# hkbharath/MARL-MASS

Measured on AMD Instinct MI355X. Metric: agent-steps/sec (whole node), MASS CBF shield on, 65536 envs x 8 CAVs, higher is better.
Workload: dtype f64

## Files before the change

### marl-mass_amd/csrc/mm_kernels.hip

```cpp
#include <hip/hip_runtime.h>
#include <math.h>
#include <stdio.h>
#include <string.h>

#include <type_traits>

#include "mm_device.h"
#include "mm_div.h"
#include "mm_handle.h"
#define MM_COUNTS_FN __host__ __device__ inline
#include "../../include/mm_counts.h"
#include "../../include/mm_policy_wide.h"

using namespace mm;

struct DevCfg {
  int env_kind, shield, nsub, T, action_masking, auto_reset, obs_f64, N, E, debug_flags, n_hdv;
  double dt, collision_reward, high_speed_reward, headway_cost, headway_time, merging_lane_cost;
  double rs_lo, rs_hi, eta, tau;
  double inv_dt, rs_span, rs_ispan, rs_span2, rs_ispan2;
  int agent_reward;
  int steer_vel;
  int *err;
  int traffic_density, mixed_traffic, num_cav;
// ... 11 lines not shown
  uint64_t *seeds;
  long long A;
  int E, N;
};

enum {
  SW_CPSI, SW_ACCN,
  SW_AX, SW_AY, SW_AH, SW_ACPSI, SW_AGVX, SW_ASTEER, SW_ASPSI,
  SW_BX, SW_BY, SW_BH, SW_BCPSI, SW_BGVX, SW_BSTEER, SW_BSPSI,
  SW_ACC,
  SW_F_COUNT
};
enum { SW_WPK, SW_APK, SW_BPK, SW_META, SW_RES, SW_CLS, SW_I_COUNT };
struct SweepBuf {
  double *F;
  int *I;
  uint8_t *order;
  uint8_t *envf;
  uint8_t *urgent;
  long long Ep;
  int N;
};
MM_DEV double &sw_f(const SweepBuf &sb, int f, int a, long long e) { return sb.F[((long long)f * sb.N + a) * sb.Ep + e]; }
MM_DEV int &sw_i(const SweepBuf &sb, int f, int a, long long e) { return sb.I[((long long)f * sb.N + a) * sb.Ep + e]; }

enum { PB_SIN, PB_COS, PB_KX, PB_KY, PB_KH, PB_F_COUNT };
constexpr int kPoseWritten = 0x200;
struct PoseBuf {
  double *F;
  int *code;
};

#ifndef MM_TU
#define MM_TU 0
#endif

#ifdef MM_STAMPS
#define MM_STAMP_WAVES (1 << 16)
__device__ unsigned long long g_stamps_w[MM_STAMP_WAVES * 16];
__device__ unsigned long long g_stamps_s[4096 * 8];
#define SSTAMP(k)                                                                        \
  do {                                                                                   \
    unsigned long long _t = __builtin_amdgcn_s_memtime();                                \
    if ((threadIdx.x & 63) == (k)) _t_acc += _t - _t_last;                               \
    _t_last = __builtin_amdgcn_s_memtime();                                              \
  } while (0)
#define SCOUNT(k) do { if ((threadIdx.x & 63) == (k)) _t_acc += 1; } while (0)
#define STAMP(k)                                                                         \
  do {                                                                                   \
    unsigned long long _t = __builtin_amdgcn_s_memtime();                                \
    if ((threadIdx.x & 63) == (k)) _t_acc += _t - _t_last;                               \
    _t_last = __builtin_amdgcn_s_memtime();                                              \
  } while (0)
#else
#define STAMP(k) do {} while (0)
#define SSTAMP(k) do {} while (0)
#define SCOUNT(k) do {} while (0)
#endif

template <int KIND> constexpr bool kIdm = KIND == MM_ENV_HDV_V1;

struct Veh {
  double x, y, h, v, tspeed;
  double act_steer, act_acc, safe_steer, safe_acc, gvx;
  double h1x, h1vx, h2x, h2vx;
  double sang;
  int lane, tlane, sidx, crashed, hl, flags, hist_len;
  int kind;
  bool present;
};

MM_DEV int lane_id() { return threadIdx.x & 63; }
MM_DEV double shfl_d(double v, int src) { return __shfl(v, src, 64); }
MM_DEV int shfl_i(int v, int src) { return __shfl(v, src, 64); }

template <int M>
MM_DEV int dppx_i(int v) {
  static_assert(M >= 1 && M <= 15, "xor mask within a 16-lane DPP row");
  if constexpr (M == 1) return __builtin_amdgcn_update_dpp(0, v, 0xB1, 0xF, 0xF, false);
  else if constexpr (M == 2) return __builtin_amdgcn_update_dpp(0, v, 0x4E, 0xF, 0xF, false);
  else if constexpr (M == 3) return __builtin_amdgcn_update_dpp(0, v, 0x1B, 0xF, 0xF, false);
  else if constexpr (M == 7) return __builtin_amdgcn_update_dpp(0, v, 0x141, 0xF, 0xF, false);
  else if constexpr (M == 8) return __builtin_amdgcn_update_dpp(0, v, 0x128, 0xF, 0xF, false);
  else if constexpr (M == 15) return __builtin_amdgcn_update_dpp(0, v, 0x140, 0xF, 0xF, false);
  else if constexpr (M < 7) return dppx_i<7>(dppx_i<7 - M>(v));
  else if constexpr (M < 12) return dppx_i<8>(dppx_i<M - 8>(v));
  else return dppx_i<15>(dppx_i<15 - M>(v));
}
template <int M>
MM_DEV double dppx_d(double v) {
  long long b = __double_as_longlong(v);
  int lo = dppx_i<M>((int)(unsigned)(b & 0xFFFFFFFFll)), hi = dppx_i<M>((int)(b >> 32));
  return __longlong_as_double(((long long)hi << 32) | (unsigned)lo);
}
template <int M, int G, class F>
MM_DEV void for_partners_impl(F &f) {
  if constexpr (M < G) {
    f(std::integral_constant<int, M>{});
    for_partners_impl<M + 1, G>(f);
  }
}
template <int G, class F>
MM_DEV void for_partners(F f) { for_partners_impl<1, G>(f); }

template <int G> constexpr bool kPow2 = (G & (G - 1)) == 0;
#ifndef MM_ROUNDS_LITE
#define MM_ROUNDS_LITE 1
#endif
constexpr bool kRoundsLite = MM_ROUNDS_LITE != 0;
#ifndef MM_VETO_PRIOR
// ... 1032 lines not shown
#ifndef MM_MIN_WAVES
#define MM_MIN_WAVES 2
#endif
#ifndef MM_NONE_WAVES
#define MM_NONE_WAVES 3
#endif
#ifndef MM_NONE_WIDE_G
#define MM_NONE_WIDE_G 99
#endif
#ifndef MM_IPM_WAVES
#define MM_IPM_WAVES 2
#endif
#ifndef MM_IPM_CAV_WAVES
#define MM_IPM_CAV_WAVES 2
#endif
#ifndef MM_IPM_WIDE_WAVES
#define MM_IPM_WIDE_WAVES 1
#endif
#ifndef MM_SPLIT_WAVES
#define MM_SPLIT_WAVES 2
#endif
template <int G, int SHIELD, bool MIXED>
#ifndef MM_GENERAL_NONE_WAVES
#define MM_GENERAL_NONE_WAVES 3
#endif
constexpr int step_min_waves(bool ipm = false) { return SHIELD == MM_SHIELD_NONE ? (G >= MM_NONE_WIDE_G ? 2 : (MIXED ? MM_GENERAL_NONE_WAVES : MM_NONE_WAVES)) : (ipm ? (G >= 6 ? MM_IPM_WIDE_WAVES : (MIXED ? MM_IPM_WAVES : MM_IPM_CAV_WAVES)) : MM_MIN_WAVES); }
template <int G, int KIND, int SHIELD, bool MIXED, bool IPM = false, bool TRACE = false, bool SPLIT = false>
#ifndef MM_STEP_BLOCK
#define MM_STEP_BLOCK 64
#endif
__global__ __launch_bounds__(MM_STEP_BLOCK, (SPLIT ? MM_SPLIT_WAVES : step_min_waves<G, SHIELD, MIXED>(IPM))) void step_kernel(DevCfg c, DevState st, const int32_t *__restrict__ actions,
                                                   MMStepOut out, double *metrics, SweepBuf sb, int kb, PoseBuf pb) {
  constexpr bool IDM = kIdm<KIND>;
  constexpr bool LC = (KIND == MM_ENV_V1) || IDM;
  constexpr bool SHIELDED = LC && (SHIELD != MM_SHIELD_NONE);
  static_assert(!IDM || (MIXED && SHIELD == MM_SHIELD_NONE && !IPM && !SPLIT), "hdv-v1: general unshielded kernels only");
  constexpr bool MASS = (SHIELD == MM_SHIELD_MASS);
  static_assert(!IPM || SHIELDED, "the IPM mode lives in shielded kernels");
  static_assert(!SPLIT || IPM, "the split form exists for the interior-point kernels");
#ifdef MM_SERIAL_ALL
  constexpr bool kSerialOnly = true || IPM;
#else
#ifdef MM_SERIAL_MASS
  constexpr bool kSerialOnly = MIXED || MASS || IPM;
#else
  constexpr bool kSerialOnly = MIXED;
#endif
#endif
  constexpr bool kSine = SHIELDED && !SPLIT && !MIXED && !IPM && !kSerialOnly && kPow2<G> && G <= 8;
#ifndef MM_CARRY_POSE
#define MM_CARRY_POSE 1
#endif
  constexpr bool kCarry = kSine && MM_CARRY_POSE != 0;
  static_assert(kPow2<G> || MM_STEP_BLOCK == 64, "rotation layouts: one wave per workgroup");
  const long long gtid = (long long)blockIdx.x * blockDim.x + threadIdx.x;
  constexpr int kTail = kPow2<G> ? 64 : (64 / G) * G;
  const bool tail = lane_id() >= kTail;
  const int gb = kPow2<G> ? (lane_id() & ~(G - 1)) : (tail ? kTail - G : lane_id() - lane_id() % G);
  const int a = kPow2<G> ? (int)(gtid % G) : lane_id() - gb;
  const long long e = kPow2<G> ? gtid / G : (tail ? (long long)st.E : (gtid >> 6) * (64 / G) + lane_id() / G);
  const bool valid = e < st.E && a < st.N;
  const long long i = e * st.N + a;
  const long long A = st.A;
  const double dt = c.dt;

#ifdef MM_STAMPS
  unsigned long long _t_last = __builtin_amdgcn_s_memtime(), _t_acc = 0;
#endif
  Veh v;
  const bool sv = MIXED && KIND == MM_ENV_V1 && c.steer_vel != 0;
  int steps = 0, time = 0, n_merge = 0, episode = 0;
  int car_code = 0;
  long long car_kx = 0, car_ky = 0, car_kh = 0;
  double car_s = 0.0, car_c = 1.0;
  if constexpr (kCarry) {
    if (valid) {
      car_kx = __double_as_longlong(pb.F[PB_KX * A + i]); car_ky = __double_as_longlong(pb.F[PB_KY * A + i]);
      car_kh = __double_as_longlong(pb.F[PB_KH * A + i]);
      car_s = pb.F[PB_SIN * A + i]; car_c = pb.F[PB_COS * A + i]; car_code = pb.code[i];
    }
  }
  load_veh(st, i, valid, v, sv);
  if (e < st.E) {
    steps = st.I[MM_E_STEPS * st.E + e]; time = st.I[MM_E_TIME * st.E + e];
  }
  if (!MIXED && v.kind == 2) v.kind = 1;
  if (IDM && v.present) v.kind = 2;
  const bool hdv = MIXED && v.kind == 2;
  const bool ctrl = IDM ? v.present : (v.present && !hdv);
  const bool ctrl_x = IDM ? false : ctrl;
  int action = (!IDM && valid && ctrl) ? actions[i] : 1;
  if ((unsigned)action > 4u) {
    if (!SPLIT || kb == 0) atomicOr(c.err, MM_LATCH_BAD_ACTION);
    action = 1;
  }
  const unsigned present_bits = group_ballot<G>(v.present, gb);
  const unsigned ctrl_bits = group_ballot<G>(ctrl, gb);
  const int n_veh = __popc(present_bits), n_ctrl = __popc(ctrl_bits);
  if (!SPLIT || kb == 0) steps += 1;

  double cpsi = 1.0, spsi = 0.0;
  double st_t = __builtin_nan("");
  int pk_self = v.lane;
  bool carried = false;
  if constexpr (kCarry) {
    const bool hit = car_kx == __double_as_longlong(v.x) && car_ky == __double_as_longlong(v.y) && car_kh == __double_as_longlong(v.h) &&
                     (car_code >> 8) == ((kPoseWritten >> 8) | (MASS ? 1 : 0)) && (car_code & 7) == v.lane;
    carried = !__any(v.present && !hit);
    if (carried && v.present) { spsi = car_s; cpsi = car_c; pk_self = car_code & 0xFF; }
  }
  if (!carried) {
    if (v.present) mmm_sincos(v.h, &spsi, &cpsi);
    if (SHIELDED && v.present) pk_self = pose_code(v.lane, next_lane(v.lane, v.x, v.y), MASS ? corner_flags(v.x, v.y, spsi, cpsi, v.lane) : 0);
  }

  enum { C_B = 0, C_H1X = 8, C_H1VX, C_H2X, C_H2VX, C_SSTEER, C_SACC, C_TSPEED, C_A = 15, C_GU0 = 23, C_GU1 = 24, C_PRE = 25, C_MSGW = 29 };
  constexpr bool kMailbox = G <= 8 || !kPow2<G>;
  constexpr bool kPackMsg = !kPow2<G>;
  constexpr int kColdB = kMailbox ? (kPackMsg ? 29 : 30) : 25;
  constexpr bool kRoomy = false;
  constexpr int C_CPSI = kColdB + G - 1, C_GVX = C_CPSI + 1;
  constexpr int kColdN = !SHIELDED ? 15 : (kSerialOnly ? 23 : kColdB + G - 1 + (kRoomy ? 2 : 0));
  static_assert(kColdN * MM_STEP_BLOCK * 8 >= (MM_STEP_BLOCK / 64) * 64 * 30 * 4, "the obs staging must fit in the cold slots");
  __shared__ double s_cold[kColdN][MM_STEP_BLOCK];
  const int tid = threadIdx.x;
  auto cold_i = [&](int slot, int col) -> int & { return ((int *)&s_cold[slot][col])[0]; };
  if (LC) {
    s_cold[C_H1X][tid] = v.h1x; s_cold[C_H1VX][tid] = v.h1vx; s_cold[C_H2X][tid] = v.h2x; s_cold[C_H2VX][tid] = v.h2vx;
    s_cold[C_SSTEER][tid] = v.safe_steer; s_cold[C_SACC][tid] = v.safe_acc;
  }
  s_cold[C_TSPEED][tid] = v.tspeed;
  if constexpr (kRoomy) { s_cold[C_CPSI][tid] = cpsi; s_cold[C_GVX][tid] = v.gvx; }
  auto CPSI = [&]() -> double { if constexpr (kRoomy) return s_cold[C_CPSI][tid]; else return cpsi; };
  auto GVX = [&]() -> double { if constexpr (kRoomy) return s_cold[C_GVX][tid]; else return v.gvx; };
  bool env_active = IDM ? n_veh > 0 : n_ctrl > 0;
  if constexpr (SPLIT) {
    if (kb > 0) env_active = e < st.E && sb.envf[e] != 0;
  }
  STAMP(0);
  const int k_lo = SPLIT ? (kb > 0 ? kb - 1 : 0) : 0, k_hi = SPLIT ? (kb < c.nsub ? kb : c.nsub - 1) : c.nsub - 1;
  for (int k = k_lo; k <= k_hi; k++) {
    const bool head = !SPLIT || k == kb, tail = !SPLIT || k != kb;
    const bool live = env_active && v.present;
    QpTrace qt = {0, __builtin_nan(""), __builtin_nan(""), __builtin_nan(""), __builtin_nan(""),
                  __builtin_nan(""), __builtin_nan(""), __builtin_nan("")};
    int rank = 0;
    if ((SHIELDED || MIXED) && head) {
      for_partners<G>([&](auto mc) {
        constexpr int m = decltype(mc)::value;
        double px = px_d<m, G>(v.x, a);
        bool pp = px_i<m, G>((int)live, a) != 0;
        rank += (pp && (px > v.x || (px == v.x && pidx<m, G>(a) < a))) ? 1 : 0;
      });
    }
    if (head) v.tspeed = s_cold[C_TSPEED][tid];
    if (live && !hdv && head) {
      if (time % c.nsub == 0) hl_act<KIND>(v, action);
    }
    const int tl_pre = v.tlane;
    if (live && !hdv && head) controlled_act<!MIXED, kSine>(v, -1, sv, st_t);
    if (head) s_cold[C_TSPEED][tid] = v.tspeed;
    if constexpr (MIXED) { STAMP(1); }
    if constexpr (MIXED) {
      if (head && __any(hdv && live)) {
        const bool acting = hdv && live && !v.crashed;
        double koff = 0.0, koff_obst = 0.0;
        if (__any(acting && v.lane == MM_LANE_KB0)) {
          koff = kSineAmp * mmm_sin(kSinePuls * (v.x - lane_sx(MM_LANE_KB0)) + kSinePhase);
          koff_obst = kSineAmp * mmm_sin(kSinePuls * (kObstX - lane_sx(MM_LANE_KB0)) + kSinePhase);
        }
        Body self = {true, false, v.x, v.y, v.h, v.v, v.tspeed, v.lane, spsi, cpsi, koff};
        const double s_me = v.x - lane_sx(v.lane);
        NbSel n0 = {0, 0, -1, -1}, n1 = {0, 0, -1, -1};
        const LaneFrame lf0 = lane_frame(v.lane);
        if (acting && lane_after_end(v.tlane, v.x)) v.tlane = next_lane(v.tlane, v.x, v.y);
        const int my_tl = v.tlane;
        const bool lc_branch = v.lane != my_tl;
        const bool same_road = lane_road(v.lane) == lane_road(my_tl);
        const bool timer_due = !lc_branch && (1.0 < v.gvx);
        const int side = v.lane == MM_LANE_BC0 ? MM_LANE_BC1 : (v.lane == MM_LANE_BC1 ? MM_LANE_BC0 : -1);
        const bool try_mobil = acting && timer_due && side >= 0 && lane_reachable(side < 0 ? 0 : side, v.x, v.y);
        const int sl = side < 0 ? 0 : side;
        const double s_side = v.x - lane_sx(sl);
        const LaneFrame lf1 = lane_frame(sl);
        unsigned abort_mask = 0;
        for_partners<G>([&](auto mc) {
          constexpr int m = decltype(mc)::value;
          const int p = pidx<m, G>(a);
          const bool bp = px_i<m, G>((int)live, a) != 0;
          const double bx = px_d<m, G>(v.x, a), by = px_d<m, G>(v.y, a), bk = px_d<m, G>(koff, a);
          if (acting) {
            neighbour_update(lf0, s_me, bp, bx, by, bk, p, n0);
            if (try_mobil) neighbour_update(lf1, s_side, bp, bx, by, bk, p, n1);
          }
          if (__any(acting && lc_branch && same_road)) {
            Body b = {bp, false, bx, by, 0.0, px_d<m, G>(v.v, a), 0.0, px_i<m, G>(v.lane, a), px_d<m, G>(spsi, a), px_d<m, G>(cpsi, a), bk};
            if (acting && lc_branch && same_road && b.present && b.lane != my_tl) {
              const double sx = lane_sx(v.lane);
              const double d = (b.x - sx) - (v.x - sx);
              if (0 < d && d < desired_gap(self, b)) abort_mask |= 1u << p;
            }
          }
        });
        if constexpr (MIXED) { STAMP(3); }
        if (acting) {
          neighbour_update(lf0, s_me, true, kObstX, kObstY, koff_obst, 99, n0);
          if (try_mobil) neighbour_update(lf1, s_side, true, kObstX, kObstY, koff_obst, 99, n1);
        }
        auto fetch = [&](int idx, bool full) {
          Body r = {};
          const int src = gb + ((idx >= 0 && idx < G) ? idx : 0);
          r.x = shfl_d(v.x, src); r.v = shfl_d(v.v, src); r.sh = shfl_d(spsi, src); r.ch = shfl_d(cpsi, src);
          if (full) { r.tspeed = shfl_d(v.tspeed, src); r.lane = shfl_i(v.lane, src); }
          r.present = idx >= 0;
          if (idx == 99) { r.is_object = true; r.x = kObstX; r.v = 0.0; r.sh = 0.0; r.ch = 1.0; r.tspeed = 0.0; r.lane = 0; }
          return r;
        };
        const Body front0 = fetch(acting ? n0.i_front : -1, false);
        Body front1 = {}, rear1 = {};
        if (__any(try_mobil)) { front1 = fetch(try_mobil ? n1.i_front : -1, false); rear1 = fetch(try_mobil ? n1.i_rear : -1, true); }
        const double acc_f0 = acting ? idm_acceleration(self, front0) : 0.0;
        bool mobil_go = false;
        if (try_mobil) {
          const double nf_pred = idm_acceleration(rear1, self);
          if (!(nf_pred < -9.0)) {
            const double jerk = idm_acceleration(self, front1) - acc_f0 + 0.0;
            mobil_go = !(jerk < 0.1);
          }
        }
        if constexpr (MIXED) { STAMP(4); }
        if (acting && timer_due) v.gvx = 0;
        int tl_post = acting ? (lc_branch ? my_tl : (mobil_go ? side : my_tl)) : v.tlane;
        for (int round = 0; round <= st.N; round++) {
          bool hit = false;
          for_partners<G>([&](auto mc) {
            constexpr int m = decltype(mc)::value;
            const int p = pidx<m, G>(a);
            const int pk = px_i<m, G>(rank | tl_pre << 4 | tl_post << 8, a);
            const int p_tl = ((pk & 15) < rank) ? ((pk >> 8) & 7) : ((pk >> 4) & 7);
            hit = hit || (((abort_mask >> p) & 1u) && p_tl == my_tl);
          });
          const int nxt = (acting && lc_branch) ? ((same_road && hit) ? v.lane : my_tl) : tl_post;
          const bool changed = nxt != tl_post;
          tl_post = nxt;
          if (!__any(changed)) break;
        }
        if constexpr (MIXED) { STAMP(5); }
        if (acting) {
          v.tlane = tl_post;
          v.act_acc = clipd(acc_f0, -6.0, 6.0);
        }
      }
      if (head && live && (!hdv || !v.crashed)) steer_lane(v, sv && !hdv, st_t);
      if (head && hdv && live) v.gvx += dt;
    }
    if (live && head) clip_actions(v, LC && !hdv, st_t);
    STAMP(1);
    Cand cA;
    memset(&cA, 0, sizeof cA);
    const bool shield_on = SHIELDED && live && !hdv && v.hist_len >= 2;
    if (live && head) cA = predict<KIND, SHIELDED, MASS, MIXED, kSine>(v, v.act_steer, st_t, spsi, cpsi, dt, sv && !hdv);
    auto park = [&](auto base_c, const Cand &cc, double steer) {
      constexpr int base = decltype(base_c)::value;
      if constexpr (SHIELDED) {
        s_cold[base + 0][tid] = cc.x; s_cold[base + 1][tid] = cc.y; s_cold[base + 2][tid] = cc.h;
        cold_i(base + 3, tid) = cc.pk; s_cold[base + 4][tid] = cc.cpsi; s_cold[base + 5][tid] = steer;
        s_cold[base + 6][tid] = cc.gvx; s_cold[base + 7][tid] = cc.spsi;
      }
    };
    if (head) park(std::integral_constant<int, C_A>{}, cA, v.act_steer);
    STAMP(2);
    const bool needB = SHIELDED && shield_on && (v.tlane != v.lane || v.crashed || sv);
    bool haveB = false;
    auto make_B = [&]() {
      if constexpr (SHIELDED) {
        if (needB && !haveB) {
          double tB;
          double steerB = steering_control<kSine>(v.x, v.y, v.h, v.v, v.lane, tB);
          if (sv) steerB = steer_vel_command(steerB, v.sang);
          park(std::integral_constant<int, C_B>{}, predict<KIND, true, MASS, MIXED, kSine>(v, steerB, tB, spsi, CPSI(), dt, sv), steerB);
          haveB = true;
        }
      }
    };
    auto chosen = [&](bool useB) {
      if constexpr (!SHIELDED) {
        return cA;
      } else {
        const int base = useB ? C_B : C_A;
        Cand cc;
        cc.x = s_cold[base + 0][tid]; cc.y = s_cold[base + 1][tid]; cc.h = s_cold[base + 2][tid];
        cc.gvx = s_cold[base + 6][tid]; cc.cpsi = s_cold[base + 4][tid]; cc.spsi = s_cold[base + 7][tid];
        const int pk = cold_i(base + 3, tid);
        cc.pk = pk; cc.lane = pk & 7;
        return cc;
      }
    };
    if constexpr (SPLIT) {
      if (!head && live && valid) {
        v.act_acc = sw_f(sb, SW_ACCN, a, e);
        if (MIXED && hdv) {
          v.act_steer = sw_f(sb, SW_ASTEER, a, e);
          if (sw_i(sb, SW_RES, a, e) & 16) s_cold[C_H1X][tid] = sw_f(sb, SW_ACC, a, e);
        }
        s_cold[C_A + 0][tid] = sw_f(sb, SW_AX, a, e); s_cold[C_A + 1][tid] = sw_f(sb, SW_AY, a, e); s_cold[C_A + 2][tid] = sw_f(sb, SW_AH, a, e);
        cold_i(C_A + 3, tid) = sw_i(sb, SW_APK, a, e); s_cold[C_A + 4][tid] = sw_f(sb, SW_ACPSI, a, e); s_cold[C_A + 5][tid] = sw_f(sb, SW_ASTEER, a, e);
        s_cold[C_A + 6][tid] = sw_f(sb, SW_AGVX, a, e); s_cold[C_A + 7][tid] = sw_f(sb, SW_ASPSI, a, e);
        if (needB) {
          s_cold[C_B + 0][tid] = sw_f(sb, SW_BX, a, e); s_cold[C_B + 1][tid] = sw_f(sb, SW_BY, a, e); s_cold[C_B + 2][tid] = sw_f(sb, SW_BH, a, e);
          cold_i(C_B + 3, tid) = sw_i(sb, SW_BPK, a, e); s_cold[C_B + 4][tid] = sw_f(sb, SW_BCPSI, a, e); s_cold[C_B + 5][tid] = sw_f(sb, SW_BSTEER, a, e);
          s_cold[C_B + 6][tid] = sw_f(sb, SW_BGVX, a, e); s_cold[C_B + 7][tid] = sw_f(sb, SW_BSPSI, a, e);
          haveB = true;
        }
      }
    }
    double new_acc = v.act_acc;
    bool use_B = false, veto = false;
    int new_flags = v.flags;
    if constexpr (SHIELDED && !SPLIT && !kSerialOnly && kVetoPrior) {
      if ((c.debug_flags & 1) == 0 && shield_on && needB && !(v.flags & MM_FLAG_IS_LC_SAFE)) { make_B(); use_B = true; }
    }
    if constexpr (SPLIT) {
      if (head) {
        make_B();
        if constexpr (!kSerialOnly && kVetoPrior) use_B = (c.debug_flags & 1) == 0 && shield_on && needB && !(v.flags & MM_FLAG_IS_LC_SAFE);
        const int n_live = __popc(group_ballot<G>(live, gb));
        if (valid) {
          sw_i(sb, SW_META, a, e) = (live ? 1 : 0) | (shield_on ? 2 : 0) | (needB ? 4 : 0) | (hdv ? 8 : 0) | (use_B ? 16 : 0) | (v.flags & 255) << 8 | (v.hl & 255) << 16;
          if (live) {
            sw_i(sb, SW_WPK, a, e) = pk_self;
            sw_f(sb, SW_CPSI, a, e) = cpsi; sw_f(sb, SW_ACCN, a, e) = v.act_acc;
            sw_f(sb, SW_AX, a, e) = cA.x; sw_f(sb, SW_AY, a, e) = cA.y; sw_f(sb, SW_AH, a, e) = cA.h; sw_i(sb, SW_APK, a, e) = cA.pk;
            sw_f(sb, SW_ACPSI, a, e) = cA.cpsi; sw_f(sb, SW_AGVX, a, e) = cA.gvx; sw_f(sb, SW_ASTEER, a, e) = v.act_steer; sw_f(sb, SW_ASPSI, a, e) = cA.spsi;
            if (needB) {
              sw_f(sb, SW_BX, a, e) = s_cold[C_B + 0][tid]; sw_f(sb, SW_BY, a, e) = s_cold[C_B + 1][tid]; sw_f(sb, SW_BH, a, e) = s_cold[C_B + 2][tid];
              sw_i(sb, SW_BPK, a, e) = cold_i(C_B + 3, tid); sw_f(sb, SW_BCPSI, a, e) = s_cold[C_B + 4][tid]; sw_f(sb, SW_BSTEER, a, e) = s_cold[C_B + 5][tid];
              sw_f(sb, SW_BGVX, a, e) = s_cold[C_B + 6][tid]; sw_f(sb, SW_BSPSI, a, e) = s_cold[C_B + 7][tid];
            }
            sb.order[(long long)rank * sb.Ep + e] = (uint8_t)a;
          }
          if (a >= n_live) sb.order[(long long)a * sb.Ep + e] = 0xFF;
          if (a == 0) sb.envf[e] = env_active ? 1 : 0;
        }
      } else if (shield_on && valid) {
        const int res = sw_i(sb, SW_RES, a, e);
        new_acc = sw_f(sb, SW_ACC, a, e); veto = (res & 2) != 0; use_B = (res & 4) != 0; new_flags = (res >> 8) & 255;
      }
    }

    if constexpr (SHIELDED) {
     if (__any(shield_on) && (!SPLIT || head)) {
      bool serial = !SPLIT && (kSerialOnly || (c.debug_flags & 1) != 0);
      ShieldOut so;
      memset(&so, 0, sizeof so);
      if constexpr (!kSerialOnly) {
       if (!serial) {
        static_assert(!MIXED || kSerialOnly, "the parallel form is CAV-only (the twin branch needs the literal sweep)");
        bool irregular = false;
        constexpr bool count5 = G > 4;
        if constexpr (kMailbox) { s_cold[C_PRE + 0][tid] = v.x; s_cold[C_PRE + 1][tid] = v.y; s_cold[C_PRE + 2][tid] = v.h; cold_i(C_PRE + 3, tid) = pk_self; }
        double qc_h0 = 0.0, qc_h3 = 0.0, qc_d = 0.0;
        int qc_meta = 0;
        (void)qc_h0; (void)qc_h3; (void)qc_d; (void)qc_meta;
        for (int pass = 0; pass <= st.N; pass++) {
#ifdef MM_STAMPS
#ifdef MM_COUNT_ROUNDS
          if ((threadIdx.x & 63) == 13) _t_acc += (pass == 0 ? 1ull << 32 : 0ull);
#else
          if ((threadIdx.x & 63) == 13) _t_acc += 1 + (pass == 0 ? 1ull << 32 : 0ull);
#endif
#endif
          const double mine_gvx = s_cold[(use_B ? C_B : C_A) + 6][tid];
          const double h1vx_mine = s_cold[C_H1VX][tid];
          s_cold[C_GU0][tid] = slot_gu<MASS>(s_cold[C_H2VX][tid], MASS ? s_cold[C_SACC][tid] : kCbfAccLo, GVX(), dt);
// ... 144 lines not shown
                }
              }
              const bool any_run = __any(run);
              if (any_run) {
                if (run) sing = mm_qp_bottom(&q, &rs) == 0;
              }
              more = any_run || __any(!fin);
            }
            if (shield_on) so = shield_post<MASS>(c, v, ss, shield_rows<true>(c, ss, nb), qc_d, (qc_meta & 8) != 0, true);
          } else {
          if constexpr (MASS && kRoundsLite) {
            const bool slow_lc = (v.hl == 2 || v.hl == 0) && v.v < kStoppingSpeed;
            ShieldRows rr;
            double d_cur = 0.0;
            for (int round = 0; round <= st.N; round++) {
#if defined(MM_STAMPS) && defined(MM_COUNT_ROUNDS)
              if ((threadIdx.x & 63) == 13) _t_acc += 1;
#endif
              const double gu_cur = slot_gu<true>(h1vx_mine, acc_cur, mine_gvx, dt);
              const double da = shfl_d(gu_cur, src_ol), db = shfl_d(gu_cur, src_oa);
              if (ol_dyn) nb.ol_gu = da;
              if (oa_dyn) nb.oa_gu = db;
              rr = shield_rows<true>(c, ss, nb);
              d_cur = qp_exact(ss, rr);
              double acc_next = v.act_acc;
              if (shield_on) {
                if (slow_lc) acc_next = shield_post<true>(c, v, ss, rr, d_cur, true, false).acc;
                else acc_next = div_c((ss.u0 + d_cur) - ss.evx, dt, c.inv_dt);
              }
              const bool changed = __double_as_longlong(acc_next) != __double_as_longlong(acc_cur);
              acc_cur = acc_next;
              if (!__any(changed)) break;
            }
            so = shield_post<true>(c, v, ss, rr, d_cur, true, false);
          } else {
          for (int round = 0; round <= st.N; round++) {
            if (MASS) {
              const double gu_cur = slot_gu<true>(h1vx_mine, acc_cur, mine_gvx, dt);
              const double da = shfl_d(gu_cur, src_ol), db = shfl_d(gu_cur, src_oa);
              if (ol_dyn) nb.ol_gu = da;
              if (oa_dyn) nb.oa_gu = db;
            }
            so = shield_dyn<MASS, true, false>(c, v, ss, nb, shield_on);
            const double acc_next = shield_on ? so.acc : v.act_acc;
            const bool changed = __double_as_longlong(acc_next) != __double_as_longlong(acc_cur);
            acc_cur = acc_next;
            if (!MASS || !__any(changed)) break;
          }
          }
          }
          if (TRACE && shield_on) trace_status(out.trace + (long long)k * MM_T_COUNT * A + i, A, so);
          STAMP(4);
          const bool want_B = shield_on && so.veto && needB;
          if (want_B) make_B();
          STAMP(5);
          const bool flip = want_B != use_B;
          use_B = want_B;
          if (!__any(flip)) break;
        }
        serial = __any(irregular);
        if (!serial && shield_on) {
          new_acc = so.acc; veto = so.veto; new_flags = so.flags; qt = so.qt;
          if (IPM && so.bounds) atomicOr(c.err, MM_LATCH_QP_BOUNDS);
        }
       }
      }
      if (!SPLIT && serial) {
        make_B();
        use_B = false; veto = false; new_acc = v.act_acc; new_flags = v.flags;
        if constexpr (kRoomy) { v.gvx = GVX(); cpsi = CPSI(); }
        double wx = v.x, wy = v.y, wh = v.h, wg = hdv ? 1.0 : v.gvx, wacc = hdv ? kCbfAccLo : s_cold[C_SACC][tid], wvx = v.v * cpsi;
        double whx = s_cold[C_H2X][tid], whvx = s_cold[C_H2VX][tid];
        int wpk = pk_self;
        if (MIXED && hdv && live) {
        }
        double wgu = slot_gu<MASS>(whvx, MASS ? wacc : kCbfAccLo, wg, dt);
        bool w_stepped = false;
        double twin_shift = 0;
        int srank = 0;
        for_partners<G>([&](auto mc) {
          constexpr int m = decltype(mc)::value;
          srank += (px_i<m, G>(shield_on ? rank : 99, a) < rank) ? 1 : 0;
        });
        for (int j = 0; j < st.N; j++) {
          const unsigned sel = group_ballot<G>(shield_on && srank == j, gb);
          if (!__any(sel != 0)) break;
          const bool has = sel != 0;
          const int ai = has ? (__ffs((int)sel) - 1) : 0;
          const int src = gb + ai;
          if constexpr (MIXED) {
            const int r_ego = shfl_i(rank, src);
            if (live && hdv && has && rank < r_ego && !w_stepped) {
              const Cand ca = chosen(false);
              wx = ca.x; wy = ca.y; wh = ca.h; wpk = ca.pk;
              whx = s_cold[C_H1X][tid]; whvx = s_cold[C_H1VX][tid]; w_stepped = true; twin_shift = 0;
              wgu = slot_gu<MASS>(whvx, MASS ? wacc : kCbfAccLo, wg, dt);
            }
          }
          const double ex = shfl_d(v.x, src), ey = shfl_d(v.y, src);
          const int epk = shfl_i(pk_self, src);
          const double e_vx = shfl_d(v.v * cpsi, src);
          const Rel rl = relate(ex, ey, epk, live && has && a != ai, wx, wy, wh, wpk, hdv);
          int pos = 0;
          for_partners<G>([&](auto mc) {
            constexpr int m = decltype(mc)::value;
            double kp = px_d<m, G>(rl.key, a);
            pos += (kp < rl.key || (kp == rl.key && pidx<m, G>(a) < a)) ? 1 : 0;
          });
          const bool in5 = rl.key < INFINITY && pos < 5;
          const unsigned none = 0x3FFu;
          unsigned f_ol = (in5 && rl.cls == 1) ? ((unsigned)pos << 5 | (unsigned)a << 1) : none;
          unsigned f_oa = (in5 && rl.cls == 2) ? ((unsigned)pos << 5 | (unsigned)a << 1 | (rl.cflag ? 1u : 0u)) : none;
          unsigned f_oar = (in5 && rl.cls == 3) ? ((unsigned)pos << 5 | (unsigned)a << 1) : none;
          const bool is_twin = MIXED && in5 && rl.cls == 4;
          if (is_twin) { whx = whx + 0.5 * e_vx; twin_shift = 1; }
          unsigned f_tw = is_twin ? ((unsigned)(15 - pos) << 5 | (unsigned)a << 1) : none;
          unsigned w = f_ol | f_oa << 10 | f_oar << 20;
          auto red = [&](auto mc) {
            constexpr int m = decltype(mc)::value;
            const unsigned o = (unsigned)dppx_i<m>((int)w);
            const unsigned m0 = min(w & 0x3FFu, o & 0x3FFu), m1 = min((w >> 10) & 0x3FFu, (o >> 10) & 0x3FFu),
// ... 7 lines not shown
            if constexpr (G >= 8) red(std::integral_constant<int, 7>{});
            if constexpr (G >= 16) red(std::integral_constant<int, 8>{});
          } else {
            auto ring = [&](auto mc) {
              constexpr int off = decltype(mc)::value;
              if constexpr (off < G) {
                const unsigned o = (unsigned)px_i<off, G>((int)w, a);
                const unsigned m0 = min(w & 0x3FFu, o & 0x3FFu), m1 = min((w >> 10) & 0x3FFu, (o >> 10) & 0x3FFu),
                               m2 = min((w >> 20) & 0x3FFu, (o >> 20) & 0x3FFu);
                w = m0 | m1 << 10 | m2 << 20;
                if (MIXED) f_tw = min(f_tw, (unsigned)px_i<off, G>((int)f_tw, a));
              }
            };
            ring(std::integral_constant<int, 1>{}); ring(std::integral_constant<int, 2>{});
            ring(std::integral_constant<int, 4>{}); ring(std::integral_constant<int, 8>{});
          }
          f_ol = w & 0x3FFu; f_oa = (w >> 10) & 0x3FFu; f_oar = (w >> 20) & 0x3FFu;
          const bool has_tw = MIXED && f_tw != none;
          if (has_tw) f_oa = f_tw & ~1u;
          Neigh nb;
          nb.has_ol = f_ol != none; nb.has_oa = f_oa != none; nb.has_oar = f_oar != none;
          const int s_ol = gb + (nb.has_ol ? (int)((f_ol >> 1) & 15u) : 0);
          const int s_oa = gb + (nb.has_oa ? (int)((f_oa >> 1) & 15u) : 0);
          const int s_oar = gb + (nb.has_oar ? (int)((f_oar >> 1) & 15u) : 0);
          nb.ol_x = shfl_d(whx, s_ol); nb.ol_gu = shfl_d(wgu, s_ol);
          nb.oa_x = shfl_d(whx, s_oa); nb.oa_gu = shfl_d(wgu, s_oa);
          nb.ol_vx = nb.oa_vx = nb.ol_acc = nb.ol_g = nb.oa_acc = nb.oa_g = 0;
          nb.oar_x = shfl_d(wx, s_oar); nb.oar_vx = shfl_d(wvx, s_oar);
          nb.constrain_adj = MASS && nb.has_oa && (f_oa & 1u);
          bool hss_collab = false;
          if (has_tw) { nb.constrain_adj = MASS; hss_collab = !MASS; }
          obstacle_override<MASS>(nb, v.x, v.y);
          const bool mine = has && a == ai && shield_on;
          ShieldOut s1 = shield_eval<MASS, true, IPM>(c, v, cpsi, pk_self, nb, mine);
          if (hss_collab) s1.flags |= MM_FLAG_IS_COLLABORATING;
          if (IPM && mine && s1.bounds) atomicOr(c.err, MM_LATCH_QP_BOUNDS);
          if (mine) {
            new_acc = s1.acc; veto = s1.veto; new_flags = s1.flags; qt = s1.qt;
            if (TRACE) trace_status(out.trace + (long long)k * MM_T_COUNT * A + i, A, s1);
            use_B = veto && needB;
            const Cand cc = chosen(use_B);
            double nv = v.v + new_acc * dt;
            nv = nv > 0 ? nv : 0;
            wx = cc.x; wy = cc.y; wh = cc.h; wg = cc.gvx; wacc = new_acc; wvx = nv * cc.cpsi;
            whx = s_cold[C_H1X][tid]; whvx = s_cold[C_H1VX][tid]; wpk = cc.pk;
            wgu = slot_gu<MASS>(whvx, MASS ? wacc : kCbfAccLo, wg, dt);
          }
        }
        if (MIXED && hdv && twin_shift != 0 && w_stepped) s_cold[C_H1X][tid] = whx;
      }
     }
    }
    STAMP(6);
    if (SPLIT && SHIELDED && out.trace && live && tail && !shield_on) {
      out.trace[(long long)k * MM_T_COUNT * A + i + MM_T_QP_ROWS * A] = 0;
    }
    if (!SPLIT && SHIELDED && TRACE && live) {
      double *t = out.trace + (long long)k * MM_T_COUNT * A + i;
      t[MM_T_QP_ROWS * A] = qt.rows; t[MM_T_QP_A * A] = qt.a;
      t[MM_T_QP_H0 * A] = qt.h0; t[MM_T_QP_H1 * A] = qt.h1; t[MM_T_QP_H2 * A] = qt.h2;
      t[MM_T_QP_H3 * A] = qt.h3; t[MM_T_QP_D * A] = qt.d; t[MM_T_LC_MARGIN * A] = qt.margin;
    }
    if (tail) {
    if (live) {
      const Cand cc = chosen(use_B);
      const double acc = (SHIELDED && shield_on) ? new_acc : v.act_acc;
      double nv = v.v + acc * dt;
      nv = nv > 0 ? nv : 0;
      if (SHIELDED && shield_on) {
        if (veto) v.tlane = v.lane;
        v.flags = new_flags;
      }
      v.x = cc.x; v.y = cc.y; v.h = cc.h; v.v = nv; v.lane = cc.lane;
      if (LC) {
        if (!hdv) {
          double steer_nom = v.act_steer;
          if constexpr (SHIELDED) steer_nom = s_cold[C_A + 5][tid];
          s_cold[C_SSTEER][tid] = (SHIELDED && shield_on && veto && haveB) ? s_cold[C_B + 5][tid] : steer_nom;
          s_cold[C_SACC][tid] = acc; v.gvx = cc.gvx;
          if constexpr (kRoomy) s_cold[C_GVX][tid] = cc.gvx;
          if (sv) v.sang += s_cold[C_SSTEER][tid] * dt;
        }
        s_cold[C_H2X][tid] = s_cold[C_H1X][tid]; s_cold[C_H2VX][tid] = s_cold[C_H1VX][tid];
        s_cold[C_H1X][tid] = v.x; s_cold[C_H1VX][tid] = v.v * cc.cpsi;
        if (v.hist_len < 2) v.hist_len++;
      }
      if constexpr (kRoomy) s_cold[C_CPSI][tid] = cc.cpsi;
      else cpsi = cc.cpsi;
      spsi = cc.spsi;
      if (SHIELDED) pk_self = cc.pk;
    }

    STAMP(7);
    unsigned need = 0;
    for_partners<G>([&](auto mc) {
      constexpr int m = decltype(mc)::value;
      double px = px_d<m, G>(v.x, a), py = px_d<m, G>(v.y, a), ph = px_d<m, G>(v.h, a);
      bool pp = px_i<m, G>((int)live, a) != 0;
      double dx = px - v.x, dy = py - v.y;
      const bool near = live & pp & !((dx * dx + dy * dy) > kU5);
      need |= (near & boxes_may_touch(dx, dy, v.h, ph, 0.9 * kVehLength / 2, 0.9 * kVehWidth / 2)) ? 1u << pidx<m, G>(a) : 0u;
    });
    {
      double dx = kObstX - v.x, dy = kObstY - v.y;
      const bool near = live & !((dx * dx + dy * dy) > kU5);
      need |= (near & boxes_may_touch(dx, dy, v.h, 0.0, 0.9 * 2.0 / 2, 0.9 * 2.0 / 2)) ? 1u << G : 0u;
// ... 249 lines not shown
    const bool spawn = valid && (c.traffic_density > 0 ? a < nc + nh : v.present);
    if (spawn) nm = spawn_vehicle(nv, a, nc, nh, seed, (uint32_t)episode);
    if (c.traffic_density > 0 && valid) {
      if (!spawn) {
        if (v.present) {
          Veh z;
          memset(&z, 0, sizeof z);
          store_veh(st, i, z, true);
        }
        v.present = false; v.kind = 0;
      }
      st.B[MM_B_KIND * A + i] = spawn ? (uint8_t)nv.kind : (uint8_t)0;
    }
    if (spawn) {
      v = nv;
      spsi = 0.0; cpsi = 1.0;
      if constexpr (kCarry) {
        mmm_sincos(v.h, &car_s, &car_c);
        pk_self = pose_code(v.lane, next_lane(v.lane, v.x, v.y), MASS ? corner_flags(v.x, v.y, car_s, car_c, v.lane) : 0);
      }
      s_cold[C_H1X][tid] = v.h1x; s_cold[C_H1VX][tid] = v.h1vx; s_cold[C_H2X][tid] = v.h2x; s_cold[C_H2VX][tid] = v.h2vx;
      s_cold[C_SSTEER][tid] = v.safe_steer; s_cold[C_SACC][tid] = v.safe_acc; s_cold[C_TSPEED][tid] = v.tspeed;
    }
    n_merge = shfl_i(nm, gb);
    steps = 0; time = 0; episode += 1;
  }
  if (valid && v.present) {
    if (LC) {
      v.h1x = s_cold[C_H1X][tid]; v.h1vx = s_cold[C_H1VX][tid]; v.h2x = s_cold[C_H2X][tid]; v.h2vx = s_cold[C_H2VX][tid];
      if (!hdv) { v.safe_steer = s_cold[C_SSTEER][tid]; v.safe_acc = s_cold[C_SACC][tid]; }
    }
    v.tspeed = s_cold[C_TSPEED][tid];
    store_veh(st, i, v, sv);
    if constexpr (kCarry) {
      pb.F[PB_KX * A + i] = v.x; pb.F[PB_KY * A + i] = v.y; pb.F[PB_KH * A + i] = v.h;
      pb.F[PB_SIN * A + i] = car_s; pb.F[PB_COS * A + i] = car_c;
      pb.code[i] = (pk_self & 0xFF) | (MASS ? 0x100 : 0) | kPoseWritten;
    }
  }
  if (e < st.E && a == 0) {
    st.I[MM_E_STEPS * st.E + e] = steps; st.I[MM_E_TIME * st.E + e] = time;
    st.I[MM_E_N_MERGE * st.E + e] = n_merge; st.I[MM_E_EPISODE * st.E + e] = episode;
  }
  STAMP(11);
  __syncthreads();
  STAMP(14);
  const double sc_h[2] = {spsi, cpsi};
  observe<G, KIND, true>(c, v, a, gb, i, valid, out.obs, out.action_mask, (float *)&s_cold[0][0], sc_h);
  STAMP(12);
#ifdef MM_STAMPS
  {
    const long long wv = gtid >> 6;
    if ((threadIdx.x & 63) < 16 && wv < MM_STAMP_WAVES) g_stamps_w[wv * 16 + (threadIdx.x & 63)] += _t_acc;
  }
#endif
}

template <int G, int KIND>
__global__ __launch_bounds__(256) void reset_kernel(DevCfg c, DevState st, int mode, const uint8_t *env_mask,
                                                    const uint64_t *seeds_in, void *obs, uint8_t *avail) {
  const long long gtid = (long long)blockIdx.x * blockDim.x + threadIdx.x;
  const long long e = gtid / G;
  const int a = (int)(gtid % G);
  const int gb = lane_id() & ~(G - 1);
  const bool valid = e < st.E && a < st.N;
  const long long i = e * st.N + a;
  const bool selected = e < st.E && mode != 2 && (!env_mask || env_mask[e]);
  Veh v;
  load_veh(st, i, valid, v);
  if (kIdm<KIND> && v.present) v.kind = 2;
  if (selected) {
    int steps = 0, time = 0, n_merge = 0, episode = st.I[MM_E_EPISODE * st.E + e];
    if (mode == 0) {
      if (seeds_in && a == 0) st.seeds[e] = seeds_in[e];
      const uint64_t seed = seeds_in ? seeds_in[e] : st.seeds[e];
      int nm = 0;
      int nc = st.N - c.n_hdv, nh = c.n_hdv;
      if (kIdm<KIND>) { nc = 0; nh = st.N; }
      episode_counts<KIND>(c, seed, (uint32_t)episode, nc, nh);
      if (valid) {
        if (a < nc + nh) nm = spawn_vehicle(v, a, nc, nh, seed, (uint32_t)episode);
        else {
          const bool was = v.present;
          memset(&v, 0, sizeof v);
          if (was) store_veh(st, i, v, true);
          v.hl = MM_HL_NONE;
        }
        st.B[MM_B_KIND * st.A + i] = (uint8_t)v.kind;
      }
      n_merge = shfl_i(nm, gb);
      episode += 1;
    } else {
      if (valid && v.present) init_vehicle(v);
      if (kIdm<KIND> && valid && v.present) st.B[MM_B_KIND * st.A + i] = 2;
      n_merge = __popc(group_ballot<G>(valid && v.kind == 1 && (v.lane == MM_LANE_JK0 || v.lane == MM_LANE_KB0), gb));
    }
    if (valid && v.present) store_veh(st, i, v, true);
    if (a == 0) {
      st.I[MM_E_STEPS * st.E + e] = steps; st.I[MM_E_TIME * st.E + e] = time;
      st.I[MM_E_N_MERGE * st.E + e] = n_merge; st.I[MM_E_EPISODE * st.E + e] = episode;
    }
  }
  observe<G, KIND>(c, v, a, gb, i, valid, obs, avail);
}


// ... 1065 lines not shown
      const double u = u53(w4[0], w4[1]);
      int a = 0;
#pragma unroll
      for (int o = 0; o < 8; o++)
        if (o < n_a) a += (cdf[o] / acc <= u) ? 1 : 0;
      actions[ag] = a < n_a - 1 ? a : n_a - 1;
    }
  }
}
extern "C" int32_t mm_policy_act(const float *obs, int64_t n, int32_t n_s, const float *W1, const float *b1, const float *W2,
                                 const float *b2, const float *W3, const float *b3, int32_t hidden, int32_t n_a, uint64_t seed,
                                 uint64_t *counter, int32_t *actions, float *logp, MMStream stream) {
  if (!obs || !W1 || !b1 || !W2 || !b2 || !W3 || !b3 || !counter || !actions) return MM_ERR_INVALID_ARG;
  if (hidden == 512)
    return mm_policy_wide_act(obs, n, n_s, W1, b1, W2, b2, W3, b3, hidden, n_a, seed, counter, actions, logp, stream);
  if (n < 0 || n_s < 1 || n_s > 32 || hidden != kPolHidden || n_a < 1 || n_a > 8) return MM_ERR_INVALID_ARG;
  if (n == 0) return MM_OK;
  hipStream_t s = (hipStream_t)stream;
  const long long ntiles = (n + 31) / 32;
  constexpr int kW = kPolThreads / 64;
  const unsigned grid = (unsigned)(ntiles < kW * 256 ? (ntiles + kW - 1) / kW : 256);
  hipLaunchKernelGGL(policy_kernel, dim3(grid), dim3(kPolThreads), 0, s, obs, (long long)n, (int)n_s, W1, b1, W2, b2, W3, b3, (int)n_a,
                     seed, counter, actions, logp);
  hipLaunchKernelGGL(bump_kernel, dim3(1), dim3(1), 0, s, counter);
  return hipGetLastError() == hipSuccess ? MM_OK : MM_ERR_DEVICE;
}

#ifdef MM_STAMPS
extern "C" int32_t mm_debug_read_sweep_stamps(unsigned long long *out8, int32_t reset) {
  static unsigned long long host[4096 * 8];
  hipError_t rc = hipMemcpyFromSymbol(host, HIP_SYMBOL(g_stamps_s), sizeof host);
  for (int k = 0; k < 8; k++) out8[k] = 0;
  for (int w = 0; w < 4096; w++)
    for (int k = 0; k < 8; k++) out8[k] += host[w * 8 + k];
  if (rc == hipSuccess && reset) {
    memset(host, 0, sizeof host);
    rc = hipMemcpyToSymbol(HIP_SYMBOL(g_stamps_s), host, sizeof host);
  }
  return rc == hipSuccess ? MM_OK : MM_ERR_DEVICE;
}
extern "C" int32_t mm_debug_read_stamps(unsigned long long *out16, int32_t reset) {
  static unsigned long long *host = nullptr;
  if (!host) host = (unsigned long long *)malloc(sizeof(unsigned long long) * MM_STAMP_WAVES * 16);
  hipError_t rc = hipMemcpyFromSymbol(host, HIP_SYMBOL(g_stamps_w), sizeof(unsigned long long) * MM_STAMP_WAVES * 16);
  for (int k = 0; k < 16; k++) out16[k] = 0;
  for (long long w = 0; w < MM_STAMP_WAVES; w++)
    for (int k = 0; k < 16; k++) out16[k] += host[w * 16 + k];
  if (rc == hipSuccess && reset) {
    memset(host, 0, sizeof(unsigned long long) * MM_STAMP_WAVES * 16);
    rc = hipMemcpyToSymbol(HIP_SYMBOL(g_stamps_w), host, sizeof(unsigned long long) * MM_STAMP_WAVES * 16);
  }
  return rc == hipSuccess ? MM_OK : MM_ERR_DEVICE;
}
#endif
#endif
```

Baseline: 2.304 billion.

## Predict the prior-held candidate first and build the other one lazily

```diff
diff --git a/marl-mass_amd/csrc/mm_kernels.hip b/marl-mass_amd/csrc/mm_kernels.hip
--- a/marl-mass_amd/csrc/mm_kernels.hip
+++ b/marl-mass_amd/csrc/mm_kernels.hip
@@ -87,10 +87,25 @@
     if ((threadIdx.x & 63) == (k)) _t_acc += _t - _t_last;                               \
     _t_last = __builtin_amdgcn_s_memtime();                                              \
   } while (0)
+enum { MM_CS_UPFRONT_CYCLES = 16,
+       MM_CS_UPFRONT,
+       MM_CS_LAZY_B,
+       MM_CS_FALLBACK,
+       MM_CS_PRIOR_HELD,
+       MM_CS_PRIOR_LIFTED,
+       MM_CS_LAZY_A,
+       MM_CS_FIRST_B };
+__device__ unsigned long long g_stamps_c[MM_STAMP_WAVES * 16];
+#define CAND_COUNT(k, cond)                                                                                  \
+  do {                                                                                                       \
+    const unsigned long long _m = __ballot(cond);                                                            \
+    if ((threadIdx.x & 63) == (k)) _t_acc += (unsigned long long)__popcll(_m) + (_m ? 1ull << 32 : 0ull);    \
+  } while (0)
 #else
 #define STAMP(k) do {} while (0)
 #define SSTAMP(k) do {} while (0)
 #define SCOUNT(k) do {} while (0)
+#define CAND_COUNT(k, cond) do {} while (0)
 #endif
 
 template <int KIND> constexpr bool kIdm = KIND == MM_ENV_HDV_V1;
@@ -1229,6 +1244,10 @@
 #define MM_CARRY_POSE 1
 #endif
   constexpr bool kCarry = kSine && MM_CARRY_POSE != 0;
+#ifndef MM_PRIMARY_PRIOR
+#define MM_PRIMARY_PRIOR 1
+#endif
+  constexpr bool kPrimary = kSine && !TRACE && kVetoPrior && MM_PRIMARY_PRIOR != 0;
   static_assert(kPow2<G> || MM_STEP_BLOCK == 64, "rotation layouts: one wave per workgroup");
   const long long gtid = (long long)blockIdx.x * blockDim.x + threadIdx.x;
   constexpr int kTail = kPow2<G> ? 64 : (64 / G) * G;
@@ -1335,7 +1354,7 @@
       if (time % c.nsub == 0) hl_act<KIND>(v, action);
     }
     const int tl_pre = v.tlane;
-    if (live && !hdv && head) controlled_act<!MIXED, kSine>(v, -1, sv, st_t);
+    if (live && !hdv && head) controlled_act<!MIXED && !kPrimary, kSine>(v, -1, sv, st_t);
     if (head) s_cold[C_TSPEED][tid] = v.tspeed;
     if constexpr (MIXED) { STAMP(1); }
     if constexpr (MIXED) {
@@ -1431,7 +1450,21 @@
       if (head && live && (!hdv || !v.crashed)) steer_lane(v, sv && !hdv, st_t);
       if (head && hdv && live) v.gvx += dt;
     }
-    if (live && head) clip_actions(v, LC && !hdv, st_t);
+    bool first_B = false;
+    if constexpr (kPrimary) {
+      static_assert(!MIXED && !SPLIT, "kPrimary: no HDVs, no steer_vel, every launch a whole step");
+      first_B = (c.debug_flags & 1) == 0 && live && v.hist_len >= 2 && (v.tlane != v.lane || v.crashed) && !(v.flags & MM_FLAG_IS_LC_SAFE);
+      if (live) {
+        const int tl_1 = v.tlane + (first_B ? v.lane - v.tlane : 0);
+        const double steer = steering_control<kSine>(v.x, v.y, v.h, v.v, tl_1, st_t);
+        v.act_steer = clipd(steer, -kPi / 3, kPi / 3);
+        const double steer_1 = v.act_steer, st_t_1 = st_t;
+        clip_actions(v, LC, st_t);
+        if (first_B) { v.act_steer = steer_1; st_t = st_t_1; }
+      }
+    } else {
+      if (live && head) clip_actions(v, LC && !hdv, st_t);
+    }
     STAMP(1);
     Cand cA;
     memset(&cA, 0, sizeof cA);
@@ -1445,10 +1478,33 @@
         s_cold[base + 6][tid] = cc.gvx; s_cold[base + 7][tid] = cc.spsi;
       }
     };
-    if (head) park(std::integral_constant<int, C_A>{}, cA, v.act_steer);
+    auto park_at = [&](int base, const Cand &cc, double steer) {
+      s_cold[base + 0][tid] = cc.x; s_cold[base + 1][tid] = cc.y; s_cold[base + 2][tid] = cc.h;
+      cold_i(base + 3, tid) = cc.pk; s_cold[base + 4][tid] = cc.cpsi; s_cold[base + 5][tid] = steer;
+      s_cold[base + 6][tid] = cc.gvx; s_cold[base + 7][tid] = cc.spsi;
+    };
+    if constexpr (kPrimary) park_at(first_B ? (int)C_B : (int)C_A, cA, v.act_steer);
+    else if (head) park(std::integral_constant<int, C_A>{}, cA, v.act_steer);
     STAMP(2);
     const bool needB = SHIELDED && shield_on && (v.tlane != v.lane || v.crashed || sv);
-    bool haveB = false;
+    bool haveB = first_B, haveA = !first_B;
+    (void)haveA;
+    auto make_other = [&]() {
+      if constexpr (kPrimary) {
+        const bool mk_A = !haveA;
+        if (mk_A || (needB && !haveB)) {
+          double t_o;
+          const int tl_o = v.lane + (mk_A ? v.tlane - v.lane : 0);
+          double steer_o = steering_control<kSine>(v.x, v.y, v.h, v.v, tl_o, t_o);
+          if (mk_A) {
+            steer_o = clipd(steer_o, -kPi / 3, kPi / 3);
+            if (v.crashed) { steer_o = 0; t_o = 0; }
+          }
+          park_at(mk_A ? (int)C_A : (int)C_B, predict<KIND, true, MASS, MIXED, kSine>(v, steer_o, t_o, spsi, cpsi, dt, false), steer_o);
+          haveA = true; haveB = haveB || !mk_A;
+        }
+      }
+    };
     auto make_B = [&]() {
       if constexpr (SHIELDED) {
         if (needB && !haveB) {
@@ -1494,9 +1550,23 @@
     double new_acc = v.act_acc;
     bool use_B = false, veto = false;
     int new_flags = v.flags;
-    if constexpr (SHIELDED && !SPLIT && !kSerialOnly && kVetoPrior) {
+#ifdef MM_STAMPS
+    bool st_prior = false;
+#endif
+    if constexpr (kPrimary) {
+      use_B = first_B;
+#ifdef MM_STAMPS
+      st_prior = first_B;
+#endif
+      CAND_COUNT(MM_CS_FIRST_B, first_B);
+    } else if constexpr (SHIELDED && !SPLIT && !kSerialOnly && kVetoPrior) {
+      CAND_COUNT(MM_CS_UPFRONT, (c.debug_flags & 1) == 0 && shield_on && needB && !(v.flags & MM_FLAG_IS_LC_SAFE));
       if ((c.debug_flags & 1) == 0 && shield_on && needB && !(v.flags & MM_FLAG_IS_LC_SAFE)) { make_B(); use_B = true; }
-    }
+#ifdef MM_STAMPS
+      st_prior = use_B;
+#endif
+    }
+    STAMP(MM_CS_UPFRONT_CYCLES);
     if constexpr (SPLIT) {
       if (head) {
         make_B();
@@ -1747,7 +1817,13 @@
           if (TRACE && shield_on) trace_status(out.trace + (long long)k * MM_T_COUNT * A + i, A, so);
           STAMP(4);
           const bool want_B = shield_on && so.veto && needB;
-          if (want_B) make_B();
+          CAND_COUNT(MM_CS_LAZY_B, want_B && !haveB);
+          if constexpr (kPrimary) {
+            CAND_COUNT(MM_CS_LAZY_A, !want_B && !haveA);
+            if (want_B ? !haveB : !haveA) make_other();
+          } else {
+            if (want_B) make_B();
+          }
           STAMP(5);
           const bool flip = want_B != use_B;
           use_B = want_B;
@@ -1761,7 +1837,9 @@
        }
       }
       if (!SPLIT && serial) {
-        make_B();
+        CAND_COUNT(MM_CS_FALLBACK, !haveA || (needB && !haveB));
+        if constexpr (kPrimary) make_other();
+        else make_B();
         use_B = false; veto = false; new_acc = v.act_acc; new_flags = v.flags;
         if constexpr (kRoomy) { v.gvx = GVX(); cpsi = CPSI(); }
         double wx = v.x, wy = v.y, wh = v.h, wg = hdv ? 1.0 : v.gvx, wacc = hdv ? kCbfAccLo : s_cold[C_SACC][tid], wvx = v.v * cpsi;
@@ -1875,6 +1953,8 @@
      }
     }
     STAMP(6);
+    CAND_COUNT(MM_CS_PRIOR_HELD, st_prior && use_B);
+    CAND_COUNT(MM_CS_PRIOR_LIFTED, st_prior && !use_B);
     if (SPLIT && SHIELDED && out.trace && live && tail && !shield_on) {
       out.trace[(long long)k * MM_T_COUNT * A + i + MM_T_QP_ROWS * A] = 0;
     }
@@ -2230,6 +2310,7 @@
   {
     const long long wv = gtid >> 6;
     if ((threadIdx.x & 63) < 16 && wv < MM_STAMP_WAVES) g_stamps_w[wv * 16 + (threadIdx.x & 63)] += _t_acc;
+    else if ((threadIdx.x & 63) < 32 && wv < MM_STAMP_WAVES) g_stamps_c[wv * 16 + (threadIdx.x & 63) - 16] += _t_acc;
   }
 #endif
 }
@@ -3401,5 +3482,23 @@
   }
   return rc == hipSuccess ? MM_OK : MM_ERR_DEVICE;
 }
-#endif
-#endif
+extern "C" int32_t mm_debug_read_cand_stamps(unsigned long long *out32, int32_t reset) {
+  static unsigned long long *host = nullptr;
+  if (!host) host = (unsigned long long *)malloc(sizeof(unsigned long long) * MM_STAMP_WAVES * 16);
+  hipError_t rc = hipMemcpyFromSymbol(host, HIP_SYMBOL(g_stamps_c), sizeof(unsigned long long) * MM_STAMP_WAVES * 16);
+  for (int k = 0; k < 32; k++) out32[k] = 0;
+  for (long long w = 0; w < MM_STAMP_WAVES; w++)
+    for (int k = 0; k < 16; k++) {
+      const unsigned long long x = host[w * 16 + k];
+      if (k == MM_CS_UPFRONT_CYCLES - 16) { out32[k] += x; continue; }
+      out32[k] += x & 0xFFFFFFFFull;
+      out32[16 + k] += x >> 32;
+    }
+  if (rc == hipSuccess && reset) {
+    memset(host, 0, sizeof(unsigned long long) * MM_STAMP_WAVES * 16);
+    rc = hipMemcpyToSymbol(HIP_SYMBOL(g_stamps_c), host, sizeof(unsigned long long) * MM_STAMP_WAVES * 16);
+  }
+  return rc == hipSuccess ? MM_OK : MM_ERR_DEVICE;
+}
+#endif
+#endif
```

After: 2.429 billion (median of 6 runs). +5.4%, better.
